# LouisRouss/DiffuLab

Hardware: AMD Instinct MI355X
Metric: train images/sec/node (DiT-S/2 flow-matching, 256x256 latents) (higher is better)
Workload: dtype bf16

## Files before the change

diffulab_amd/csrc/gemm_rows_body.h:

```cpp
#ifndef DIFFULAB_GEMM_ROWS_BODY_H
#define DIFFULAB_GEMM_ROWS_BODY_H

#include "common.h"

typedef __attribute__((address_space(3))) void lds_void_t;
typedef const __attribute__((address_space(1))) void glb_void_t;

static __device__ __forceinline__ void glds16_s(const void* sbase, uint32_t voff, const void* lds_dst_wave_base) {
  uint32_t keep;
  const uint32_t dst = (uint32_t)(uintptr_t)(lds_void_t*)lds_dst_wave_base;
  asm volatile("s_nop 4\n\ts_mov_b32 %0, m0\n\ts_mov_b32 m0, %3\n\ts_nop 0\n\tglobal_load_lds_dwordx4 %1, %2\n\ts_mov_b32 m0, %0"
               : "=&s"(keep)
               : "v"(voff), "s"(sbase), "s"(dst)
               : "memory");
}

#define RK_BM 256
#define RK_BN 384
#define RK_BK 64
#define RK_THREADS 512
#define RK_STAGE ((RK_BM + RK_BN) * 128)
#define RK_CH 10
#define RK_JN 6
#define RK_PITCH 784
#define RK_D8 48

enum { RK_LNF = 0, RK_LNB = 1, RK_QK = 2 };

struct RowEpi {
  const bf16_t* resid;
  const bf16_t* gate;
  int64_t ld_gate;
  const float* ln_w;
  const float* ln_b;
  const bf16_t* scale;
  const bf16_t* shift;
  int64_t ld_mod;
  float eps;
  bf16_t* t_out;
  bf16_t* x_out;
  bf16_t* xm_out;
  float* mean;
  float* rstd;
  const bf16_t* x;
  const float* mean_i;
  const float* rstd_i;
  const bf16_t* dres;
  bf16_t* dx;
  float* dscale;
  float* dshift;
  int64_t ld_dmod;
  float* dwb;
  const bf16_t* gt;
  bf16_t* gdt;
  float* dgate;
  bf16_t* qkv;
  bf16_t* qo;
  bf16_t* ko;
  float* rrms;
  const float* sq;
  const float* sk;
  const float* cs;
  const float* sn;
  int n_tok, heads, dh, rot, n_dst, n_off;
};

template <int N>
static __device__ __forceinline__ void rk_wait_vmcnt() {
  asm volatile("s_waitcnt vmcnt(%0)" ::"n"(N) : "memory");
}
static __device__ __forceinline__ void rk_lds_barrier() {
  asm volatile("s_waitcnt lgkmcnt(0)" ::: "memory");
  __builtin_amdgcn_s_barrier();
  asm volatile("" ::: "memory");
}

static __device__ __forceinline__ u32x4_t rk_ld16(const bf16_t* p) { return *(const u32x4_t*)p; }

template <int MODE>
static __device__ __forceinline__ void rk_row_epilogue(uint32_t (&P)[RK_JN][2][8], char* lds, int tile_m, int tile_n, int lane,
                                                       int wave, const RowEpi& ep) {
  constexpr int D = RK_BN;
  const int hi = lane >> 5, wm = wave >> 1, wn = wave & 1;
  const bool on = lane < RK_D8;
  const int64_t m0 = (int64_t)tile_m * RK_BM;
  const int64_t g = tile_m;
  const float invD = 1.0f / (float)D;
  const int c8 = lane * 8;

  float k0[8], k1[8], k2[8], k3[8], k4[8];
#pragma unroll
  for (int e = 0; e < 8; ++e) k0[e] = k1[e] = k2[e] = k3[e] = k4[e] = 0.f;
  if constexpr (MODE == RK_LNF) {
    if (on) {
      if (ep.ln_w) {
        *(f32x4_t*)&k0[0] = *(const f32x4_t*)(ep.ln_w + c8);
        *(f32x4_t*)&k0[4] = *(const f32x4_t*)(ep.ln_w + c8 + 4);
        *(f32x4_t*)&k1[0] = *(const f32x4_t*)(ep.ln_b + c8);
        *(f32x4_t*)&k1[4] = *(const f32x4_t*)(ep.ln_b + c8 + 4);
      } else {
#pragma unroll
        for (int e = 0; e < 8; ++e) k0[e] = 1.0f;
      }
      unpack8(rk_ld16(ep.scale + g * ep.ld_mod + c8), k2);
      unpack8(rk_ld16(ep.shift + g * ep.ld_mod + c8), k3);
      if (ep.gate) unpack8(rk_ld16(ep.gate + g * ep.ld_gate + c8), k4);
    } else {
#pragma unroll
      for (int e = 0; e < 8; ++e) k0[e] = 1.0f;
    }
  } else if constexpr (MODE == RK_LNB) {
    if (on) {
      float wv[8], sc[8];
#pragma unroll
      for (int e = 0; e < 8; ++e) wv[e] = 1.0f;
      if (ep.ln_w) {
        *(f32x4_t*)&wv[0] = *(const f32x4_t*)(ep.ln_w + c8);
        *(f32x4_t*)&wv[4] = *(const f32x4_t*)(ep.ln_w + c8 + 4);
      }
      unpack8(rk_ld16(ep.scale + g * ep.ld_mod + c8), sc);
#pragma unroll
      for (int e = 0; e < 8; ++e) k0[e] = (1.0f + sc[e]) * wv[e];
      if (ep.gt) unpack8(rk_ld16(ep.gate + g * ep.ld_gate + c8), k4);
    } else {
#pragma unroll
      for (int e = 0; e < 8; ++e) k0[e] = 1.0f;
    }
  } else {
    if (on && tile_n < 2) {
      const float* s = tile_n == 0 ? ep.sq : ep.sk;
      *(f32x4_t*)&k0[0] = *(const f32x4_t*)(s + c8);
      *(f32x4_t*)&k0[4] = *(const f32x4_t*)(s + c8 + 4);
    }
  }

  u32x4_t pa = {0, 0, 0, 0}, pb = {0, 0, 0, 0}, pc = {0, 0, 0, 0};
  float pf0 = 0.f, pf1 = 0.f;
  auto row_of = [&](int s) -> int64_t {
    const int i = s >> 4, pair = (s >> 3) & 1, lr = (s & 7) * 8 + wave;
    return m0 + (2 * pair + (lr >> 5)) * 64 + i * 32 + (lr & 31);
  };
  auto fetch = [&](int s) {
    const int64_t row = row_of(s);
    if constexpr (MODE == RK_LNF) {
      if (on && ep.resid) pa = rk_ld16(ep.resid + row * D + c8);
    } else if constexpr (MODE == RK_LNB) {
      if (on) {
        pa = rk_ld16(ep.x + row * D + c8);
        if (ep.dres) pb = rk_ld16(ep.dres + row * D + c8);
        if (ep.gt) pc = rk_ld16(ep.gt + row * D + c8);
      }
      pf0 = ep.mean_i[row];
      pf1 = ep.rstd_i[row];
    } else {
      if (on && tile_n < 2) {
        const int dh = ep.dh, h = c8 / dh, d0 = c8 - h * dh;
        if (d0 < ep.rot) {
          const int n = (int)(row % ep.n_tok);
          const f32x4_t cc = *(const f32x4_t*)(ep.cs + (int64_t)n * (ep.rot >> 1) + (d0 >> 1));
          const f32x4_t ss = *(const f32x4_t*)(ep.sn + (int64_t)n * (ep.rot >> 1) + (d0 >> 1));
          pa = __builtin_bit_cast(u32x4_t, cc);
          pb = __builtin_bit_cast(u32x4_t, ss);
        }
      }
    }
  };

  fetch(0);
  rk_lds_barrier();
#pragma unroll
  for (int i = 0; i < 2; ++i) {
    for (int pair = 0; pair < 2; ++pair) {
      if ((wm >> 1) == pair) {
        char* base = lds + ((wm & 1) * 32 + (lane & 31)) * RK_PITCH + (wn * 192 + 8 * hi) * 2;
#pragma unroll
        for (int j = 0; j < RK_JN; ++j)
#pragma unroll
          for (int gp = 0; gp < 2; ++gp) {
            const auto s0 = __builtin_amdgcn_permlane32_swap(P[j][i][4 * gp + 0], P[j][i][4 * gp + 2], false, false);
            const auto s1 = __builtin_amdgcn_permlane32_swap(P[j][i][4 * gp + 1], P[j][i][4 * gp + 3], false, false);
            u32x4_t v = {s0[0], s1[0], s0[1], s1[1]};
            *(u32x4_t*)(base + (j * 32 + 16 * gp) * 2) = v;
          }
      }
      rk_lds_barrier();
      for (int rr = 0; rr < 8; ++rr) {
        const int s = (i * 2 + pair) * 8 + rr;
        const int lr = rr * 8 + wave;
        const int64_t row = row_of(s);
        const u32x4_t qa = pa, qb = pb, qc = pc;
        const float f0 = pf0, f1 = pf1;
        if (s + 1 < 32) fetch(s + 1);
        u32x4_t tq = {0, 0, 0, 0};
        if (on) tq = *(const u32x4_t*)(lds + lr * RK_PITCH + lane * 16);
        float tv[8];
        unpack8(tq, tv);

        if constexpr (MODE == RK_LNF) {
          if (on && ep.t_out) *(u32x4_t*)(ep.t_out + row * D + c8) = tq;
          float xv[8];
          if (ep.resid) {
            unpack8(qa, xv);
            if (ep.gate) {
#pragma unroll
              for (int e = 0; e < 8; ++e) xv[e] = bf2f(f2bf(xv[e] + k4[e] * tv[e]));
            } else {
#pragma unroll
              for (int e = 0; e < 8; ++e) xv[e] = bf2f(f2bf(xv[e] + tv[e]));
            }
          } else {
#pragma unroll
            for (int e = 0; e < 8; ++e) xv[e] = tv[e];
          }
          if (on && ep.x_out) *(u32x4_t*)(ep.x_out + row * D + c8) = pack8(xv);
          float sm = 0.f;
#pragma unroll
          for (int e = 0; e < 8; ++e) sm += xv[e];
          const float mu = wave_sum(sm) * invD;
          float q = 0.f;
#pragma unroll
          for (int e = 0; e < 8; ++e) {
            const float d = on ? (xv[e] - mu) : 0.f;
            q += d * d;
          }
          const float rs = rsqrtf(wave_sum(q) * invD + ep.eps);
#pragma unroll
          for (int e = 0; e < 8; ++e) {
            const float y = (xv[e] - mu) * rs * k0[e] + k1[e];
            xv[e] = y * (1.0f + k2[e]) + k3[e];
          }
          if (on) *(u32x4_t*)(ep.xm_out + row * D + c8) = pack8(xv);
          if (lane == 0) {
            ep.mean[row] = mu;
            ep.rstd[row] = rs;
          }
        } else if constexpr (MODE == RK_LNB) {
          float xv[8], rv[8];
          unpack8(qa, xv);
#pragma unroll
          for (int e = 0; e < 8; ++e) rv[e] = 0.f;
          if (ep.dres) unpack8(qb, rv);
          const float mu = f0, rs = f1;
          float s1 = 0.f, s2 = 0.f;
#pragma unroll
          for (int e = 0; e < 8; ++e) {
            const float xh = on ? (xv[e] - mu) * rs : 0.f;
            const float d = tv[e];
            k1[e] += d;
            k2[e] += d * xh;
            const float dxh = d * k0[e];
            s1 += dxh;
            s2 += dxh * xh;
            xv[e] = xh;
            tv[e] = dxh;
          }
          const float c1 = wave_sum(s1) * invD, c2 = wave_sum(s2) * invD;
#pragma unroll
          for (int e = 0; e < 8; ++e) rv[e] += rs * (tv[e] - c1 - xv[e] * c2);
          if (on) *(u32x4_t*)(ep.dx + row * D + c8) = pack8(rv);
          if (ep.gt) {
            float gtv[8];
            unpack8(qc, gtv);
#pragma unroll
            for (int e = 0; e < 8; ++e) {
              const float dxr = bf2f(f2bf(rv[e]));
              k3[e] += on ? dxr * gtv[e] : 0.f;
              rv[e] = dxr * k4[e];
            }
            if (on) *(u32x4_t*)(ep.gdt + row * D + c8) = pack8(rv);
          }
        } else {
          if (on) *(u32x4_t*)(ep.qkv + row * (3 * D) + tile_n * D + c8) = tq;
          if (tile_n < 2) {
            float s1 = 0.f;
#pragma unroll
            for (int e = 0; e < 8; ++e) s1 += tv[e] * tv[e];
            const float rq = rsqrtf(wave_sum(s1) * invD + ep.eps);
            if (on) {
              const int dh = ep.dh, h = c8 / dh, d0 = c8 - h * dh;
#pragma unroll
              for (int e = 0; e < 8; ++e) tv[e] = tv[e] * rq * k0[e];
              if (d0 < ep.rot) {
                const f32x4_t cc = __builtin_bit_cast(f32x4_t, qa), ss = __builtin_bit_cast(f32x4_t, qb);
#pragma unroll
                for (int p = 0; p < 4; ++p) {
                  const float a = tv[2 * p], b = tv[2 * p + 1];
                  tv[2 * p] = a * cc[p] - b * ss[p];
                  tv[2 * p + 1] = a * ss[p] + b * cc[p];
                }
              }
              const int64_t bb = row / ep.n_tok;
              const int n = (int)(row - bb * ep.n_tok);
              const int64_t o = ((bb * ep.heads + h) * ep.n_dst + ep.n_off + n) * dh + d0;
              *(u32x4_t*)((tile_n == 0 ? ep.qo : ep.ko) + o) = pack8(tv);
            }
            if (lane == 0) ep.rrms[row * 2 + tile_n] = rq;
          }
        }
      }
      rk_lds_barrier();
    }
  }

  if constexpr (MODE == RK_LNB) {
    float* red = (float*)lds;
    if (on) {
      float* slot = red + (size_t)wave * 3 * D + c8;
      *(f32x4_t*)(slot) = *(f32x4_t*)&k1[0];
      *(f32x4_t*)(slot + 4) = *(f32x4_t*)&k1[4];
      *(f32x4_t*)(slot + D) = *(f32x4_t*)&k2[0];
      *(f32x4_t*)(slot + D + 4) = *(f32x4_t*)&k2[4];
      *(f32x4_t*)(slot + 2 * D) = *(f32x4_t*)&k3[0];
      *(f32x4_t*)(slot + 2 * D + 4) = *(f32x4_t*)&k3[4];
    }
    rk_lds_barrier();
    const int col = threadIdx.x;
    if (col < D) {
      float S1 = 0.f, S2 = 0.f, S3 = 0.f;
#pragma unroll
      for (int w = 0; w < 8; ++w) {
        S1 += red[(size_t)w * 3 * D + col];
        S2 += red[(size_t)w * 3 * D + D + col];
        S3 += red[(size_t)w * 3 * D + 2 * D + col];
      }
      const float wc = ep.ln_w ? ep.ln_w[col] : 1.0f, bc = ep.ln_b ? ep.ln_b[col] : 0.0f;
      const float sc1 = 1.0f + bf2f(ep.scale[g * ep.ld_mod + col]);
      ep.dscale[g * ep.ld_dmod + col] = wc * S2 + bc * S1;
      ep.dshift[g * ep.ld_dmod + col] = S1;
      if (ep.gt) ep.dgate[g * ep.ld_dmod + col] = S3;
      if (ep.dwb) {
        ep.dwb[(size_t)g * 2 * D + col] = sc1 * S2;
        ep.dwb[(size_t)g * 2 * D + D + col] = sc1 * S1;
      }
    }
    rk_lds_barrier();
  }
}

template <int MODE>
static __device__ __forceinline__ void rk_gemm_body(const bf16_t* __restrict__ A, int64_t lda, const bf16_t* __restrict__ Bm,
                                                    int64_t ldb, int N, int K, const RowEpi& ep, char* smem, int tid, int first,
                                                    int stride, int cnt) {
  const int lane = tid & 63, hi = lane >> 5;
  const int wave = __builtin_amdgcn_readfirstlane(tid >> 6);
  const int wm = wave >> 1, wn = wave & 1;
  const int tiles_n = N / RK_BN;
  const int nk = K / RK_BK;
  const int total = cnt * nk;

  int s_tile = first, s_kt = 0, s_it = 0;
  const bf16_t* s_ta = A + (int64_t)((s_tile / tiles_n) * RK_BM) * lda;
  const bf16_t* s_tb = Bm + (int64_t)((s_tile % tiles_n) * RK_BN) * ldb;

  f32x16_t acc[RK_JN][2];
#pragma unroll
  for (int j = 0; j < RK_JN; ++j)
#pragma unroll
    for (int i = 0; i < 2; ++i)
#pragma unroll
      for (int r = 0; r < 16; ++r) acc[j][i][r] = 0.f;

  int it = 0;
  for (int t = 0; t < cnt; ++t) {
    const int tile = first + t * stride;
    int ln = lane;
    asm volatile("" : "+v"(ln));
    const int lhi = ln >> 5;
    uint32_t src_off[RK_CH];
    int lds_off[RK_CH];
    bool is_a[RK_CH];
#pragma unroll
    for (int i = 0; i < RK_CH; ++i) {
      const int c = wave * RK_CH + i;
      is_a[i] = c < RK_BM / 8;
      const int cc = is_a[i] ? c : c - RK_BM / 8;
      const int r = cc * 8 + (ln >> 3);
      const int q = (ln & 7) ^ ((r >> 1) & 7);
      src_off[i] = (uint32_t)(r * (int)(is_a[i] ? lda : ldb) + q * 8) * 2u;
      lds_off[i] = (is_a[i] ? 0 : RK_BM * 128) + cc * 1024;
    }
    auto stage_next = [&]() {
      char* base = smem + (s_it & 1) * RK_STAGE;
      const char* ka = (const char*)(s_ta + s_kt * RK_BK);
      const char* kb = (const char*)(s_tb + s_kt * RK_BK);
#pragma unroll
      for (int i = 0; i < RK_CH; ++i) glds16_s(is_a[i] ? ka : kb, src_off[i], base + lds_off[i]);
      ++s_it;
      if (++s_kt == nk) {
        s_kt = 0;
        s_tile += stride;
        s_ta = A + (int64_t)((s_tile / tiles_n) * RK_BM) * lda;
        s_tb = Bm + (int64_t)((s_tile % tiles_n) * RK_BN) * ldb;
      }
    };
    int xrow[2], wrow[RK_JN];
#pragma unroll
    for (int i = 0; i < 2; ++i) xrow[i] = wm * 64 + i * 32 + (ln & 31);
#pragma unroll
    for (int j = 0; j < RK_JN; ++j) wrow[j] = wn * (RK_BN / 2) + j * 32 + (ln & 31);

    if (t == 0) stage_next();
    for (int kt = 0; kt < nk; ++kt, ++it) {
      rk_wait_vmcnt<0>();
      __builtin_amdgcn_s_barrier();
      if (s_it < total) stage_next();
      const char* sa = smem + (it & 1) * RK_STAGE;
      const char* sb = sa + RK_BM * 128;
      bf16x8_t xq[2][2], wq[3];
      auto rd_x = [&](int kk, int i) -> bf16x8_t {
        return *(const bf16x8_t*)(sa + xrow[i] * 128 + ((((kk << 1) | lhi) ^ ((xrow[i] >> 1) & 7)) << 4));
      };
      auto rd_w = [&](int kk, int j) -> bf16x8_t {
        return *(const bf16x8_t*)(sb + wrow[j] * 128 + ((((kk << 1) | lhi) ^ ((wrow[j] >> 1) & 7)) << 4));
      };
      xq[0][0] = rd_x(0, 0);
      xq[0][1] = rd_x(0, 1);
      wq[0] = rd_w(0, 0);
      wq[1] = rd_w(0, 1);
#pragma unroll
      for (int s = 0; s < 4 * RK_JN; ++s) {
        const int kk = s / RK_JN, j = s % RK_JN;
        __builtin_amdgcn_sched_barrier(0);
        if (s + 2 < 4 * RK_JN) wq[(s + 2) % 3] = rd_w((s + 2) / RK_JN, (s + 2) % RK_JN);
        if (kk < 3 && j < 2) xq[(kk + 1) & 1][j] = rd_x(kk + 1, j);
#pragma unroll
        for (int i = 0; i < 2; ++i) acc[j][i] = __builtin_amdgcn_mfma_f32_32x32x16_bf16(wq[s % 3], xq[kk & 1][i], acc[j][i], 0, 0, 0);
      }
      __builtin_amdgcn_sched_barrier(0);
    }
    uint32_t P[RK_JN][2][8];
#pragma unroll
    for (int j = 0; j < RK_JN; ++j)
#pragma unroll
      for (int i = 0; i < 2; ++i) {
#pragma unroll
        for (int q = 0; q < 8; ++q) P[j][i][q] = pack2bf(acc[j][i][2 * q], acc[j][i][2 * q + 1]);
#pragma unroll
        for (int r = 0; r < 16; ++r) acc[j][i][r] = 0.f;
      }
    rk_row_epilogue<MODE>(P, smem + ((it - 1) & 1) * RK_STAGE, tile / tiles_n, tile % tiles_n, lane, wave, ep);
  }
}

#endif
```

Before: 12870.

## Split LNF row epilogue into specialized kernel with prefetch ring and uniform lanes

Moves the residual+gate+LayerNorm+modulation epilogue out of the generic row epilogue into a dedicated routine. The new routine is templated on whether t_out and x_out exist, and prefetches residual rows through an 8-deep register ring. Off-range lanes duplicate work instead of branching, and per-row mean/rstd are gathered into lane registers and written once at the end. The aim is to hide global-load latency and remove divergent branches and scalar stores in the epilogue. The cost is higher register pressure and an fp-contract-controlled sum of squares that may shift rounding slightly.

```diff
diff --git a/diffulab_amd/csrc/gemm_rows_body.h b/diffulab_amd/csrc/gemm_rows_body.h
--- a/diffulab_amd/csrc/gemm_rows_body.h
+++ b/diffulab_amd/csrc/gemm_rows_body.h
@@ -91,25 +91,7 @@
   float k0[8], k1[8], k2[8], k3[8], k4[8];
 #pragma unroll
   for (int e = 0; e < 8; ++e) k0[e] = k1[e] = k2[e] = k3[e] = k4[e] = 0.f;
-  if constexpr (MODE == RK_LNF) {
-    if (on) {
-      if (ep.ln_w) {
-        *(f32x4_t*)&k0[0] = *(const f32x4_t*)(ep.ln_w + c8);
-        *(f32x4_t*)&k0[4] = *(const f32x4_t*)(ep.ln_w + c8 + 4);
-        *(f32x4_t*)&k1[0] = *(const f32x4_t*)(ep.ln_b + c8);
-        *(f32x4_t*)&k1[4] = *(const f32x4_t*)(ep.ln_b + c8 + 4);
-      } else {
-#pragma unroll
-        for (int e = 0; e < 8; ++e) k0[e] = 1.0f;
-      }
-      unpack8(rk_ld16(ep.scale + g * ep.ld_mod + c8), k2);
-      unpack8(rk_ld16(ep.shift + g * ep.ld_mod + c8), k3);
-      if (ep.gate) unpack8(rk_ld16(ep.gate + g * ep.ld_gate + c8), k4);
-    } else {
-#pragma unroll
-      for (int e = 0; e < 8; ++e) k0[e] = 1.0f;
-    }
-  } else if constexpr (MODE == RK_LNB) {
+  if constexpr (MODE == RK_LNB) {
     if (on) {
       float wv[8], sc[8];
 #pragma unroll
@@ -142,9 +124,7 @@
   };
   auto fetch = [&](int s) {
     const int64_t row = row_of(s);
-    if constexpr (MODE == RK_LNF) {
-      if (on && ep.resid) pa = rk_ld16(ep.resid + row * D + c8);
-    } else if constexpr (MODE == RK_LNB) {
+    if constexpr (MODE == RK_LNB) {
       if (on) {
         pa = rk_ld16(ep.x + row * D + c8);
         if (ep.dres) pb = rk_ld16(ep.dres + row * D + c8);
@@ -196,45 +176,7 @@
         float tv[8];
         unpack8(tq, tv);
 
-        if constexpr (MODE == RK_LNF) {
-          if (on && ep.t_out) *(u32x4_t*)(ep.t_out + row * D + c8) = tq;
-          float xv[8];
-          if (ep.resid) {
-            unpack8(qa, xv);
-            if (ep.gate) {
-#pragma unroll
-              for (int e = 0; e < 8; ++e) xv[e] = bf2f(f2bf(xv[e] + k4[e] * tv[e]));
-            } else {
-#pragma unroll
-              for (int e = 0; e < 8; ++e) xv[e] = bf2f(f2bf(xv[e] + tv[e]));
-            }
-          } else {
-#pragma unroll
-            for (int e = 0; e < 8; ++e) xv[e] = tv[e];
-          }
-          if (on && ep.x_out) *(u32x4_t*)(ep.x_out + row * D + c8) = pack8(xv);
-          float sm = 0.f;
-#pragma unroll
-          for (int e = 0; e < 8; ++e) sm += xv[e];
-          const float mu = wave_sum(sm) * invD;
-          float q = 0.f;
-#pragma unroll
-          for (int e = 0; e < 8; ++e) {
-            const float d = on ? (xv[e] - mu) : 0.f;
-            q += d * d;
-          }
-          const float rs = rsqrtf(wave_sum(q) * invD + ep.eps);
-#pragma unroll
-          for (int e = 0; e < 8; ++e) {
-            const float y = (xv[e] - mu) * rs * k0[e] + k1[e];
-            xv[e] = y * (1.0f + k2[e]) + k3[e];
-          }
-          if (on) *(u32x4_t*)(ep.xm_out + row * D + c8) = pack8(xv);
-          if (lane == 0) {
-            ep.mean[row] = mu;
-            ep.rstd[row] = rs;
-          }
-        } else if constexpr (MODE == RK_LNB) {
+        if constexpr (MODE == RK_LNB) {
           float xv[8], rv[8];
           unpack8(qa, xv);
 #pragma unroll
@@ -334,6 +276,139 @@
       }
     }
     rk_lds_barrier();
+  }
+}
+
+#define RK_RING_LNF 8
+
+template <int I>
+static __device__ __forceinline__ void rk_dump_piece(uint32_t (&P)[RK_JN][2][8], char* lds, int lane, int wave) {
+  const int hi = lane >> 5, wm = wave >> 1, wn = wave & 1;
+  char* base = lds + ((wm & 1) * 32 + (lane & 31)) * RK_PITCH + (wn * 192 + 8 * hi) * 2;
+#pragma unroll
+  for (int j = 0; j < RK_JN; ++j)
+#pragma unroll
+    for (int gp = 0; gp < 2; ++gp) {
+      const auto s0 = __builtin_amdgcn_permlane32_swap(P[j][I][4 * gp + 0], P[j][I][4 * gp + 2], false, false);
+      const auto s1 = __builtin_amdgcn_permlane32_swap(P[j][I][4 * gp + 1], P[j][I][4 * gp + 3], false, false);
+      u32x4_t v = {s0[0], s1[0], s0[1], s1[1]};
+      *(u32x4_t*)(base + (j * 32 + 16 * gp) * 2) = v;
+    }
+}
+
+static __device__ __forceinline__ int rk_tile_row(int s, int wave) {
+  const int i = s >> 4, pair = (s >> 3) & 1, lr = (s & 7) * 8 + wave;
+  return (2 * pair + (lr >> 5)) * 64 + i * 32 + (lr & 31);
+}
+
+static __device__ __forceinline__ float rk_ssq8(const float (&d)[8]) {
+#pragma clang fp contract(off)
+  float q = __builtin_fmaf(d[0], d[0], d[1] * d[1]);
+#pragma unroll
+  for (int e = 2; e < 8; ++e) q = __builtin_fmaf(d[e], d[e], q);
+  return q;
+}
+
+template <bool HAS_T, bool HAS_X>
+static __device__ __forceinline__ void rk_lnf_rows(uint32_t (&P)[RK_JN][2][8], char* lds, int tile_m, int lane, int wave,
+                                                   const RowEpi& ep) {
+  constexpr int D = RK_BN, R = RK_RING_LNF;
+  static_assert(8 % R == 0, "a ring slot is a fixed register of the unrolled piece");
+  const int wm = wave >> 1;
+  asm volatile("" : "+v"(lane));
+  const bool on = lane < RK_D8;
+  const int cl = on ? lane : lane - RK_D8;
+  const int c8 = cl * 8;
+  const int64_t g = tile_m;
+  const int64_t e0 = (int64_t)tile_m * RK_BM * D;
+  const float invD = 1.0f / (float)D;
+  const bool has_resid = ep.resid != nullptr, has_gate = ep.gate != nullptr;
+
+  float k0[8], k1[8], k2[8], k3[8], k4[8];
+#pragma unroll
+  for (int e = 0; e < 8; ++e) k0[e] = 1.0f, k1[e] = 0.f, k4[e] = 1.0f;
+  if (ep.ln_w) {
+    *(f32x4_t*)&k0[0] = *(const f32x4_t*)(ep.ln_w + c8);
+    *(f32x4_t*)&k0[4] = *(const f32x4_t*)(ep.ln_w + c8 + 4);
+    *(f32x4_t*)&k1[0] = *(const f32x4_t*)(ep.ln_b + c8);
+    *(f32x4_t*)&k1[4] = *(const f32x4_t*)(ep.ln_b + c8 + 4);
+  }
+  unpack8(rk_ld16(ep.scale + g * ep.ld_mod + c8), k2);
+  unpack8(rk_ld16(ep.shift + g * ep.ld_mod + c8), k3);
+  if (has_gate) unpack8(rk_ld16(ep.gate + g * ep.ld_gate + c8), k4);
+
+  const bf16_t* src = (has_resid ? ep.resid : ep.xm_out) + e0;
+  bf16_t* const t_out = HAS_T ? ep.t_out + e0 : nullptr;
+  bf16_t* const x_out = HAS_X ? ep.x_out + e0 : nullptr;
+  bf16_t* const xm_out = ep.xm_out + e0;
+  u32x4_t ring[R];
+#pragma unroll
+  for (int r = 0; r < R; ++r) ring[r] = rk_ld16(src + (uint32_t)(rk_tile_row(r, wave) * D + c8));
+  float muv = 0.f, rsv = 0.f;
+
+  rk_lds_barrier();
+  for (int pc = 0; pc < 4; ++pc) {
+    if ((wm >> 1) == (pc & 1)) {
+      if (pc < 2)
+        rk_dump_piece<0>(P, lds, lane, wave);
+      else
+        rk_dump_piece<1>(P, lds, lane, wave);
+    }
+    rk_lds_barrier();
+#pragma unroll
+    for (int rr = 0; rr < 8; ++rr) {
+      const int s = pc * 8 + rr;
+      const uint32_t off = (uint32_t)(rk_tile_row(s, wave) * D + c8);
+      float xv[8];
+      unpack8(ring[rr % R], xv);
+      asm volatile("" : "+v"(xv[0]), "+v"(xv[1]), "+v"(xv[2]), "+v"(xv[3]), "+v"(xv[4]), "+v"(xv[5]), "+v"(xv[6]), "+v"(xv[7])::"memory");
+      const int sn = s + R < 32 ? s + R : 31;
+      ring[rr % R] = rk_ld16(src + (uint32_t)(rk_tile_row(sn, wave) * D + c8));
+      const u32x4_t tq = *(const u32x4_t*)(lds + (rr * 8 + wave) * RK_PITCH + cl * 16);
+      float tv[8];
+      unpack8(tq, tv);
+      if constexpr (HAS_T) *(u32x4_t*)(t_out + off) = tq;
+#pragma unroll
+      for (int e = 0; e < 8; ++e) xv[e] = bf2f(f2bf((has_resid ? xv[e] : -0.0f) + k4[e] * tv[e]));
+      if constexpr (HAS_X) *(u32x4_t*)(x_out + off) = pack8(xv);
+      float sm = 0.f;
+#pragma unroll
+      for (int e = 0; e < 8; ++e) sm += xv[e];
+      const float mu = wave_sum(on ? sm : 0.f) * invD;
+      float dv[8];
+#pragma unroll
+      for (int e = 0; e < 8; ++e) dv[e] = xv[e] - mu;
+      const float rs = rsqrtf(wave_sum(on ? rk_ssq8(dv) : 0.f) * invD + ep.eps);
+#pragma unroll
+      for (int e = 0; e < 8; ++e) {
+        const float y = dv[e] * rs * k0[e] + k1[e];
+        xv[e] = y * (1.0f + k2[e]) + k3[e];
+      }
+      *(u32x4_t*)(xm_out + off) = pack8(xv);
+      muv = lane == s ? mu : muv;
+      rsv = lane == s ? rs : rsv;
+    }
+    rk_lds_barrier();
+  }
+  if (lane < 32) {
+    const int64_t row = (int64_t)tile_m * RK_BM + rk_tile_row(lane, wave);
+    ep.mean[row] = muv;
+    ep.rstd[row] = rsv;
+  }
+}
+
+static __device__ __forceinline__ void rk_lnf_epilogue(uint32_t (&P)[RK_JN][2][8], char* lds, int tile_m, int lane, int wave,
+                                                       const RowEpi& ep) {
+  if (ep.t_out) {
+    if (ep.x_out)
+      rk_lnf_rows<true, true>(P, lds, tile_m, lane, wave, ep);
+    else
+      rk_lnf_rows<true, false>(P, lds, tile_m, lane, wave, ep);
+  } else {
+    if (ep.x_out)
+      rk_lnf_rows<false, true>(P, lds, tile_m, lane, wave, ep);
+    else
+      rk_lnf_rows<false, false>(P, lds, tile_m, lane, wave, ep);
   }
 }
 
@@ -438,7 +513,11 @@
 #pragma unroll
         for (int r = 0; r < 16; ++r) acc[j][i][r] = 0.f;
       }
-    rk_row_epilogue<MODE>(P, smem + ((it - 1) & 1) * RK_STAGE, tile / tiles_n, tile % tiles_n, lane, wave, ep);
+    char* piece = smem + ((it - 1) & 1) * RK_STAGE;
+    if constexpr (MODE == RK_LNF)
+      rk_lnf_epilogue(P, piece, tile / tiles_n, lane, wave, ep);
+    else
+      rk_row_epilogue<MODE>(P, piece, tile / tiles_n, tile % tiles_n, lane, wave, ep);
   }
 }
 
```

Result: no change. 12930 (median of 6 runs) (+0.5%).
